# zlib-ng/minizip-ng

Hardware: AMD Instinct MI355X
Metric: decompressed GiB/s (whole node) + CRC32 match rate, 100k x 64KiB DEFLATE entries (higher is better)
Workload: dtype u8

## Files before the change

minizip-ng_amd/csrc/crc32_core.h:

```cpp
#ifndef MZHIP_CRC32_CORE_H
#define MZHIP_CRC32_CORE_H

#include <stddef.h>
#include "wave.h"

#define MZ_CRC_POLY 0xEDB88320u
#define MZ_CRC_TILE 1024u
#define MZ_CRC_SUPER 4096u

typedef struct mzhip_crc_tables {
    uint32_t byte_tab[256];
    uint32_t kx[32];
    uint32_t x16[64];
    uint32_t x1[16];
    uint32_t kx4[32];
    uint32_t x64[64];
    uint32_t mul4[4][256];
    uint32_t slice[4][256];
} mzhip_crc_tables;

static inline uint32_t mzhip_gf2_mul_host(uint32_t a, uint32_t b) {
    uint32_t p = 0;
    for (int i = 0; i < 32; i++) {
        if (a & 0x80000000u) p ^= b;
        a <<= 1;
        b = (b & 1) ? ((b >> 1) ^ MZ_CRC_POLY) : (b >> 1);
    }
    return p;
}
static inline uint32_t mzhip_xpow8_host(uint64_t nbytes) {
    uint32_t r = 0x80000000u, sq = 0x00800000u;
    while (nbytes) {
        if (nbytes & 1) r = mzhip_gf2_mul_host(r, sq);
        sq = mzhip_gf2_mul_host(sq, sq);
        nbytes >>= 1;
    }
    return r;
}
static inline void mzhip_crc_tables_init(mzhip_crc_tables *t) {
    for (uint32_t n = 0; n < 256; n++) {
        uint32_t c = n;
        for (int k = 0; k < 8; k++) c = (c & 1) ? (MZ_CRC_POLY ^ (c >> 1)) : (c >> 1);
        t->byte_tab[n] = c;
    }
    uint32_t k = mzhip_xpow8_host(MZ_CRC_TILE - 16);
    for (int j = 0; j < 32; j++) {
        t->kx[j] = k;
        k = (k & 1) ? ((k >> 1) ^ MZ_CRC_POLY) : (k >> 1);
    }
    for (int j = 0; j < 64; j++) t->x16[j] = mzhip_xpow8_host(16u * (uint32_t)j);
    for (int j = 0; j < 16; j++) t->x1[j] = mzhip_xpow8_host((uint32_t)j);
    k = mzhip_xpow8_host(MZ_CRC_SUPER - 64);
    for (int j = 0; j < 32; j++) {
        t->kx4[j] = k;
        k = (k & 1) ? ((k >> 1) ^ MZ_CRC_POLY) : (k >> 1);
    }
    for (int j = 0; j < 64; j++) t->x64[j] = mzhip_xpow8_host(64u * (uint32_t)j);
    for (int b = 0; b < 4; b++)
        for (uint32_t n = 0; n < 256; n++) t->mul4[b][n] = mzhip_gf2_mul_host(n << (8 * b), t->kx4[0]);
    for (uint32_t n = 0; n < 256; n++) t->slice[0][n] = t->byte_tab[n];
    for (int k2 = 1; k2 < 4; k2++)
        for (uint32_t n = 0; n < 256; n++) t->slice[k2][n] = (t->slice[k2 - 1][n] >> 8) ^ t->byte_tab[t->slice[k2 - 1][n] & 255];
}
static inline uint32_t mzhip_crc32_combine_host(uint32_t crc_a, uint32_t crc_b, uint64_t len_b) {
    return mzhip_gf2_mul_host(mzhip_xpow8_host(len_b), crc_a) ^ crc_b;
}

MZ_DEV uint32_t mz_gf2_mul(uint32_t a, uint32_t b) {
    uint32_t p = 0;
#pragma unroll 4
    for (int i = 0; i < 32; i++) {
        p ^= b & (0u - (a >> 31));
        a <<= 1;
        b = (b >> 1) ^ (MZ_CRC_POLY & (0u - (b & 1)));
    }
    return p;
}

MZ_DEV uint32_t mz_gf2_mul_kx(uint32_t a, const uint32_t *kx) {
    uint32_t p = 0;
#pragma unroll
    for (int j = 0; j < 32; j++)
        p ^= kx[j] & (0u - ((a >> (31 - j)) & 1u));
    return p;
}

MZ_DEV uint32_t mz_load_u32(const uint8_t *p) {
    uint32_t v;
    __builtin_memcpy(&v, p, 4);
    return v;
}

MZ_DEV uint32_t mz_crc_dword(uint32_t r, uint32_t d, const uint32_t *tab) {
    r ^= d;
    r = tab[r & 255] ^ (r >> 8);
    r = tab[r & 255] ^ (r >> 8);
    r = tab[r & 255] ^ (r >> 8);
    r = tab[r & 255] ^ (r >> 8);
    return r;
}

#define MZ_CRC_FOLD_TILES(acc, done, buf, upto, tab, kx)                                   \
    while ((uint64_t)(done) + MZ_CRC_TILE <= (uint64_t)(upto)) {                           \
        MZ_LANES {                                                                         \
            const uint8_t *_p = (buf) + (done) + 16u * (uint32_t)lane;                     \
            uint32_t _r = P(acc);                                                          \
            if ((done) != 0) _r = mz_gf2_mul_kx(_r, (kx));      \
            _r = mz_crc_dword(_r, mz_load_u32(_p), (tab));                                 \
            _r = mz_crc_dword(_r, mz_load_u32(_p + 4), (tab));                             \
            _r = mz_crc_dword(_r, mz_load_u32(_p + 8), (tab));                             \
            _r = mz_crc_dword(_r, mz_load_u32(_p + 12), (tab));                            \
            P(acc) = _r;                                                                   \
        }                                                                                  \
        (done) += MZ_CRC_TILE;                                                             \
    }

MZ_DEV uint32_t mz_crc_dword4(uint32_t r, uint32_t d, const uint32_t *tab4) {
    const uint32_t x = r ^ d;
    return tab4[768u + (x & 255u)] ^ tab4[512u + ((x >> 8) & 255u)] ^ tab4[256u + ((x >> 16) & 255u)] ^ tab4[x >> 24];
}

#define MZ_CRC_FOLD_SUPER(acc, done, buf, n, tab4, mul4)                                    \
    while ((uint64_t)(done) + MZ_CRC_SUPER <= (uint64_t)(n)) {                             \
        MZ_LANES {                                                                         \
            const uint8_t *_p = (buf) + (done) + 64u * (uint32_t)lane;                     \
            uint32_t _r = P(acc);                                                          \
            if ((done) != 0)  \
                _r = (mul4)[_r & 255u] ^ (mul4)[256u + ((_r >> 8) & 255u)] ^ (mul4)[512u + ((_r >> 16) & 255u)] ^ (mul4)[768u + (_r >> 24)]; \
            for (int _k = 0; _k < 4; _k++) {                                               \
                uint32_t _q[4];                                                            \
                __builtin_memcpy(_q, _p + 16 * _k, 16);              \
                _r = mz_crc_dword4(_r, _q[0], (tab4));                                     \
                _r = mz_crc_dword4(_r, _q[1], (tab4));                                     \
                _r = mz_crc_dword4(_r, _q[2], (tab4));                                     \
                _r = mz_crc_dword4(_r, _q[3], (tab4));                                     \
            }                                                                              \
            P(acc) = _r;                                                                   \
        }                                                                                  \
        (done) += MZ_CRC_SUPER;                                                            \
    }
#define MZ_CRC_ADVANCE_SUPER(r, kxp) mz_crc_advance_gm((r), (const uint32_t *)((const uint8_t *)(kxp) + (offsetof(mzhip_crc_tables, mul4) - offsetof(mzhip_crc_tables, kx4))))
MZ_DEV uint32_t mz_crc_advance_gm(uint32_t r, const uint32_t *mul4) {
    return mul4[r & 255u] ^ mul4[256u + ((r >> 8) & 255u)] ^ mul4[512u + ((r >> 16) & 255u)] ^ mul4[768u + (r >> 24)];
}
#define MZ_CRC_FOLD_SUPER_BT(acc, done, buf, upto, tab, kx4)                               \
    while ((uint64_t)(done) + MZ_CRC_SUPER <= (uint64_t)(upto)) {                          \
        MZ_LANES {                                                                         \
            const uint8_t *_p = (buf) + (done) + 64u * (uint32_t)lane;                     \
            uint32_t _r = P(acc);                                                          \
            if ((done) != 0) _r = MZ_CRC_ADVANCE_SUPER(_r, (kx4));                         \
            for (int _k = 0; _k < 4; _k++) {                                               \
                uint32_t _q[4];                                                            \
                __builtin_memcpy(_q, _p + 16 * _k, 16);              \
                _r = mz_crc_dword(_r, _q[0], (tab));                                       \
                _r = mz_crc_dword(_r, _q[1], (tab));                                       \
                _r = mz_crc_dword(_r, _q[2], (tab));                                       \
                _r = mz_crc_dword(_r, _q[3], (tab));                                       \
            }                                                                              \
            P(acc) = _r;                                                                   \
        }                                                                                  \
        (done) += MZ_CRC_SUPER;                                                            \
    }
#define MZ_CRC_FINISH_SUPER_BT(result, acc, tmp, done, buf, n, tab, tabs)                  \
    do {                                                                                   \
        uint32_t _sreg = 0xFFFFFFFFu;                                                      \
        if ((done) != 0) {                                                                 \
            MZ_CRC_SUPER_REDUCE(_sreg, acc, tmp, tabs);                                    \
        }                                                                                  \
        const uint8_t *_rest = (buf) + (done);                                             \
        const uint32_t _nrest = (uint32_t)((n) - (done));                                  \
        uint32_t _rdone = 0;                                                               \
        MZ_LANES { P(acc) = (lane == 0) ? _sreg : 0u; }                                    \
        MZ_CRC_FOLD_TILES(acc, _rdone, _rest, _nrest, tab, (tabs)->kx);                    \
        MZ_CRC_FINISH_FROM(result, acc, tmp, _rdone, _rest, _nrest, tab, tabs, _sreg);     \
    } while (0)
#define MZ_CRC_SUPER_REDUCE(reg, acc, tmp, tabs)                                           \
    do {                                                                                   \
        MZ_LANES { P(tmp) = mz_gf2_mul(P(acc), (tabs)->x64[63 - lane]); }                  \
        MZ_WAVE_XOR(reg, tmp);                                                             \
    } while (0)

#define MZ_CRC_FINISH_FROM(result, acc, tmp, done, buf, n, tab, tabs, reg0)                \
    do {                                                                                   \
        uint32_t _reg = (reg0);                                                            \
        if ((done) != 0) {                                                                 \
            MZ_LANES { P(tmp) = mz_gf2_mul(P(acc), (tabs)->x16[63 - lane]); }              \
            MZ_WAVE_XOR(_reg, tmp);                                                        \
        }                                                                                  \
        uint32_t _r = (uint32_t)((n) - (done));                    \
        if (_r != 0) {                                                                     \
            MZ_LANES {                                                                     \
                uint32_t _o = 16u * (uint32_t)lane;                                        \
                uint32_t _v = _r > _o ? (_r - _o > 16u ? 16u : _r - _o) : 0u;              \
                uint32_t _c = (lane == 0) ? _reg : 0u;                                     \
                const uint8_t *_p = (buf) + (done) + _o;                                   \
                for (uint32_t _i = 0; _i < _v; _i++)                                       \
                    _c = (tab)[(_c ^ _p[_i]) & 255] ^ (_c >> 8);                           \
                uint32_t _rem = _r - _o - _v;           \
                if (_v == 0) { _c = 0; _rem = 0; }                                         \
                _c = mz_gf2_mul(_c, (tabs)->x16[_rem >> 4]);                               \
                _c = mz_gf2_mul(_c, (tabs)->x1[_rem & 15]);                                \
                P(tmp) = _c;                                                               \
            }                                                                              \
            MZ_WAVE_XOR(_reg, tmp);                                                        \
        }                                                                                  \
        (result) = ~_reg;                                                                  \
    } while (0)

#define MZ_CRC_FINISH(result, acc, tmp, done, buf, n, tab, tabs) \
    MZ_CRC_FINISH_FROM(result, acc, tmp, done, buf, n, tab, tabs, 0xFFFFFFFFu)

#endif
```

minizip-ng_amd/csrc/inflate_commit.inc:

```
{
    MZ_WAVE_SYNC();
    uint8_t *const gdst = out + out_pos;
    MZ_STAT(10, Tb); MZ_STAT(12, Tm); MZ_STAT(15, 1);
    {
        uint64_t badm;
        MZ_BALLOT(badm, P(bad) != 0u);
        if (badm) fail = 1;
    }
    uint32_t nnear = 0;
    for (uint32_t b = 0; b < Tm && !fail; b += 64u) {
        PV(uint32_t, e0);
        PV(uint32_t, rem);
        MZ_LANES {
            mz_piece32 pc;
            const uint32_t j = b + (uint32_t)lane;
            uint32_t en = 0, rm = 0, nf = 0, si = 0;
            if (j < Tm) {
                en = lst[-(int32_t)(j + 1u)];
                si = en & 0xFFFu;
                const uint32_t ln = mz_bfe(en, 12, 5) + 1u, dist = (en >> 17) + 1u;
                const uint32_t dstw = si - sb;
                if (dist > dstw) {
                    nf = dist - dstw;
                    if (nf > ln) nf = ln;
// ... 47 lines not shown
            }
            P(d0) = a;
            P(rem) = rm;
            P(dist) = ds;
            P(kst) = rm ? a : 0xFFFFFFFFu;
            P(ken) = rm ? a + rm : 0xFFFFFFFFu;
            P(ca) = 0u;
            P(cb) = 0u;
        }
#pragma unroll
        for (uint32_t step = 32u; step != 0u; step >>= 1) {
            PV(uint32_t, va);
            PV(uint32_t, vb);
            MZ_GATHER(va, ken, P(ca) + step - 1u);
            MZ_GATHER(vb, kst, P(cb) + step - 1u);
            MZ_LANES {
                const uint32_t s0 = P(d0) - P(dist), s1 = s0 + ((P(rem) < P(dist)) ? P(rem) : P(dist));
                if (P(va) <= s0) P(ca) += step;
                if (P(vb) < s1) P(cb) += step;
            }
        }
        MZ_LANES {
            P(dep) = (P(cb) > P(ca)) ? ((~0ull >> (64u - (P(cb) - P(ca)))) << P(ca)) : 0ull;
        }
        uint64_t U;
        MZ_BALLOT(U, P(rem) != 0u);
        MZ_STAT_ZERO(11);
        while (U) {
            MZ_STAT(14, 1); MZ_STAT(11, 1); MZ_STAT_MAX(24, 11);
            uint64_t R;
            MZ_BALLOT(R, P(rem) != 0u && (P(dep) & U) == 0ull);
            if (!R) {
                MZ_STAT(22, 1);
                fail = 1;
                break;
            }
            MZ_LANES {
                if (P(rem) != 0u && (P(dep) & U) == 0ull) {
                    uint8_t *d = stg + P(d0);
                    uint32_t n = P(rem), D = P(dist);
                    if (D < 8u) {
                        const uint32_t D8 = D * ((7u + D) / D);
                        uint32_t pro = D8 - D;
                        if (pro > n) pro = n;
                        for (uint32_t k = 0; k < pro; k++) d[k] = d[(int32_t)k - (int32_t)D];
                        d += pro;
                        n -= pro;
                        D = D8;
                    }
                    mz_copy32_seq(d, d - D, n);
                    P(rem) = 0u;
                }
            }
            MZ_WAVE_SYNC();
            U &= ~R;
        }
    }
#endif
    MZ_PROF_MARK(7);
    if (!fail) {
#if !(MZ_ABLATE & 8)
        {
            const uint32_t e = sb + Tb;
            const uint32_t a0 = sb ? 16u : 0u, a1 = e & ~15u;
            uint8_t *const gal = gdst - sb;
            const uint32_t hn = ((a0 < e) ? a0 : e) - sb;
            const uint32_t t0 = (a1 > a0) ? a1 : a0;
            const uint32_t tn = (e > t0) ? e - t0 : 0u;
            MZ_LANES {
                if ((uint32_t)lane < hn) gal[sb + (uint32_t)lane] = stg[sb + (uint32_t)lane];
                if ((uint32_t)lane < tn) gal[t0 + (uint32_t)lane] = stg[t0 + (uint32_t)lane];
                for (uint32_t c = a0 + 16u * (uint32_t)lane; c + 16u <= a1; c += 1024u) {
                    const uint64_t v0 = mz_ld8(stg + c), v1 = mz_ld8(stg + c + 8u);
                    mz_st8(gal + c, v0);
                    mz_st8(gal + c + 8u, v1);
                }
            }
        }
#endif
        MZ_WAVE_SYNC();
        out_pos += Tb;
        MZ_PROF_MARK(8);
#if !(MZ_ABLATE & 4)
        MZ_CRC_FOLD_SUPER_BT(crc_acc, crc_done, out + crc_base, out_pos - crc_base, crc_tab, tabs->kx4);
#endif
        MZ_PROF_MARK(9);
    }
}
```

minizip-ng_amd/csrc/inflate_core.h:

```cpp
#ifndef MZHIP_INFLATE_CORE_H
#define MZHIP_INFLATE_CORE_H
#if defined(MZ_STATS)
extern unsigned long long mz_stats[32], mz_stat_max;
#define MZ_STAT(i, v) (mz_stats[i] += (v))
#define MZ_STAT_ZERO(i) (mz_stats[i] = 0)
#define MZ_STAT_MAX(i, j) (mz_stats[i] = mz_stats[j] > mz_stats[i] ? mz_stats[j] : mz_stats[i])
#define MZ_STAT_LANE(v) (mz_stat_max = (v) > mz_stat_max ? (v) : mz_stat_max)
#define MZ_STAT_LANEMAX(i) (mz_stats[i] += mz_stat_max, mz_stat_max = 0)
#else
#define MZ_STAT(i, v) ((void)0)
#define MZ_STAT_ZERO(i) ((void)0)
#define MZ_STAT_MAX(i, j) ((void)0)
#define MZ_STAT_LANE(v) ((void)0)
#define MZ_STAT_LANEMAX(i) ((void)0)
#endif

#include "crc32_core.h"
#include "wave.h"
#if defined(MZ_PROF) && !defined(MZHIP_HOST_EMUL)
extern __device__ unsigned long long mz_prof_buf[32];
#define MZ_PROF_DECL                     \
    uint32_t prof_acc = 0;  \
    uint64_t prof_t0 = __builtin_readcyclecounter();
#define MZ_PROF_MARK(i)                                                           \
// ... 200 lines not shown
    for (int k = root + 1; k < 15; k++) len += (v15 >= lim[k]) ? 1u : 0u;
    const uint32_t idx = (uint32_t)((int32_t)delta[len] + (int32_t)(v15 >> (15u - len)));
    const uint32_t ok = (v15 < lim[15] && idx < nent) ? 1u : 0u;
    const uint32_t e = ent[ok ? idx : 0u];
    return ok ? e + len : 0u;
}

#define MZ_HDR_WIN_BITS(dst, pos_)                                                            \
    do {                                                                                      \
        const uint32_t _ab = (pos_) + 8u * in_mis, _j = (_ab >> 5) - hw0;                     \
        if (_j + 2u < 64u) {                                                                  \
            const uint32_t _d0 = MZ_READLANE(hwin, _j), _d1 = MZ_READLANE(hwin, _j + 1u), _d2 = MZ_READLANE(hwin, _j + 2u); \
            const uint32_t _s = _ab & 31u;                                                    \
            uint64_t _v = (((uint64_t)_d1 << 32) | _d0) >> _s;                                \
            if (_s) _v |= (uint64_t)_d2 << (64u - _s);                                        \
            (dst) = _v;                                                                       \
        } else {                                                                              \
            (dst) = mz_bits_at(in, in_len, (pos_));                                           \
        }                                                                                     \
    } while (0)

#define MZ_HDR_BITS(dst, n)                                                   \
    do {                                                                      \
        if (bitpos + (uint32_t)(n) > total_bits) {                            \
            status = MZHIP_BUF_ERROR;                                         \
            goto finish;                                                      \
        }                                                                     \
        uint64_t _w;                                                          \
        MZ_HDR_WIN_BITS(_w, bitpos);                                          \
        (dst) = MZ_UNIFORM((uint32_t)_w & ((1u << (n)) - 1));                 \
        bitpos += (n);                                                        \
    } while (0)

MZ_DEV uint32_t mz_load_stream_dword(const uint8_t *in_al, uint32_t in_mis, uint32_t in_len, uint32_t j) {
    const uint64_t lo = (uint64_t)j * 4u, end = (uint64_t)in_mis + in_len;
    if (lo >= end) return 0u;
    uint32_t d = *(const uint32_t *)(in_al + lo);
    if (lo < in_mis) d &= 0xFFFFFFFFu << (8u * (in_mis - (uint32_t)lo));
    if (lo + 4u > end) d &= 0xFFFFFFFFu >> (8u * (uint32_t)(lo + 4u - end));
    return d;
}

#if defined(MZHIP_HOST_EMUL)
static const uint8_t mz_k_order[19] = {16, 17, 18, 0, 8, 7, 9, 6, 10, 5, 11, 4, 12, 3, 13, 2, 14, 1, 15};
#else
__device__ static const uint8_t mz_k_order[19] = {16, 17, 18, 0, 8, 7, 9, 6, 10, 5, 11, 4, 12, 3, 13, 2, 14, 1, 15};
#endif


MZ_DEV void mz_bitrange(uint32_t sh, uint32_t n, uint32_t *m0, uint32_t *m1) {
    const uint32_t full = 0xFFFFFFFFu >> (32u - n);
    *m0 = full << sh;
    *m1 = (full >> 1) >> (31u - sh);
}
typedef struct {
    uint64_t v[4];
    uint32_t t4, t2, t1;
} mz_piece32;
MZ_DEV void mz_copy32_load(mz_piece32 *r, const uint8_t *src, uint32_t n) {
    const uint32_t n8 = n & ~7u;
    r->v[0] = r->v[1] = r->v[2] = r->v[3] = 0;
    r->t4 = r->t2 = r->t1 = 0;
#pragma unroll
    for (uint32_t k = 0; k < 4u; k++)
        if (8u * k + 8u <= n) r->v[k] = mz_ld8(src + 8u * k);
    if (n & 4u) r->t4 = mz_ld4(src + n8);
    if (n & 2u) r->t2 = mz_ld2(src + n8 + (n & 4u));
    if (n & 1u) r->t1 = src[n - 1u];
}
MZ_DEV void mz_copy32_store(const mz_piece32 *r, uint8_t *dst, uint32_t n) {
    const uint32_t n8 = n & ~7u;
#pragma unroll
    for (uint32_t k = 0; k < 4u; k++)
        if (8u * k + 8u <= n) mz_st8(dst + 8u * k, r->v[k]);
    if (n & 4u) mz_st4(dst + n8, r->t4);
    if (n & 2u) mz_st2(dst + n8 + (n & 4u), (uint16_t)r->t2);
    if (n & 1u) dst[n - 1u] = (uint8_t)r->t1;
}
MZ_DEV void mz_copy32(uint8_t *dst, const uint8_t *src, uint32_t n) {
    mz_piece32 r;
    mz_copy32_load(&r, src, n);
    mz_copy32_store(&r, dst, n);
}
MZ_DEV void mz_copy32_seq(uint8_t *dst, const uint8_t *src, uint32_t n) {
    const uint32_t n8 = n & ~7u;
#pragma unroll
    for (uint32_t k = 0; k < 4u; k++)
        if (8u * k + 8u <= n) mz_st8(dst + 8u * k, mz_ld8(src + 8u * k));
    if (n & 4u) mz_st4(dst + n8, mz_ld4(src + n8));
    if (n & 2u) mz_st2(dst + n8 + (n & 4u), mz_ld2(src + n8 + (n & 4u)));
    if (n & 1u) dst[n - 1u] = src[n - 1u];
}

#define MZ_K_LIT 0x40u
#define MZ_K_EOB 0x80u
MZ_DEV uint32_t mz_chase_step(const mz_inflate_lds *L, uint32_t d0, uint32_t d1, uint32_t d2, uint32_t rel, uint32_t room,
                              uint32_t *rec) {
    uint32_t w0 = mz_funnel(d1, d0, rel), w1 = mz_funnel(d2, d1, rel);
    uint32_t e = L->lit_fast[w0 & ((1u << MZ_LROOT) - 1u)];
    if (e & MZ_E_SUB) e = L->lit_sub[((e >> 8) & 0x1FFu) + mz_bfe(w0, MZ_LROOT, e & 7u)];
    uint32_t r = 0, pb = 0;
    if ((((e & (MZ_E_LEN | 0x80u)) == 0x80u) & ((e & 63u) < room)) != 0) {
        pb = e & 63u;
        r = 0x80000000u | mz_bfe(e, 16, 8);
        w0 = mz_funnel(w1, w0, pb);
        w1 >>= pb;
        e = L->lit_fast[w0 & ((1u << MZ_LROOT) - 1u)];
        if (e & MZ_E_SUB) e = L->lit_sub[((e >> 8) & 0x1FFu) + mz_bfe(w0, MZ_LROOT, e & 7u)];
    }
    if (!(e & MZ_E_LEN)) {
        const uint32_t nb = e & 63u;
        *rec = r | ((e >> 8) & 0xFF00u);
        return nb ? ((nb + pb) | ((e & 0x80u) ? MZ_K_LIT : MZ_K_EOB)) : 0u;
    }
    const uint32_t nb = e & 63u, ex = mz_bfe(e, 16, 4);
    const uint32_t lenl = mz_bfe(e, 7, 9) + mz_bfe(mz_funnel(w1, w0, nb), 0, ex);
    const uint32_t nb2 = nb + ex;
    const uint32_t dl = mz_funnel(w1, w0, nb2);
    uint32_t dd = L->dist_fast[dl & ((1u << MZ_DROOT) - 1u)];
    MZ_STAT(19, 1);
    if (dd == 0u) {
        MZ_STAT(20, 1);
        dd = mz_long_code(dl, MZ_DROOT, L->dist_lim, L->dist_delta, L->dist_ent, 32u);
    }
    if ((int32_t)dd <= 0) {
        *rec = 0u;
        return 0u;
    }
    const uint32_t dn = dd & 15u, dex = mz_bfe(dd, 4, 4);
    const uint32_t dist = mz_bfe(dd, 8, 15) + mz_bfe(dl, dn, dex);
    *rec = r | ((lenl - 3u) << 8) | ((dist - 1u) << 16);
    return nb2 + dn + dex + pb;
}
typedef struct { uint32_t v[4]; } mz_dw4;
MZ_DEV mz_dw4 mz_load_stream_dw4(const uint8_t *in_al, uint32_t in_mis, uint32_t in_len, uint32_t d) {
    mz_dw4 r;
    const uint64_t lo = (uint64_t)d * 4u, end = (uint64_t)in_mis + in_len;
    if (lo >= in_mis && lo + 16u <= end) {
        __builtin_memcpy(&r, in_al + lo, 16);
    } else {
#pragma unroll
        for (uint32_t k = 0; k < 4u; k++) r.v[k] = mz_load_stream_dword(in_al, in_mis, in_len, d + k);
    }
    return r;
}


#include "inflate_walk.inc"
#include "inflate_emit.inc"

typedef struct mz_inflate_par {
    uint32_t mode;
    uint32_t *ptr;
} mz_inflate_par;
#define MZHIP_PAR_BAIL (-301)

MZ_DEV uint32_t mz_block_header_plausible(const uint8_t *in, uint32_t in_len, uint32_t p) {
    if ((uint64_t)(p >> 3) + 24u > in_len) return 0u;
    uint64_t w = mz_bits_at(in, in_len, p);
    const uint32_t h = (uint32_t)w;
    if (((h >> 1) & 3u) == 0u) {
        const uint32_t b = (p + 3u + 7u) >> 3;
        const uint32_t len = (uint32_t)in[b] | ((uint32_t)in[b + 1] << 8), nlen = (uint32_t)in[b + 2] | ((uint32_t)in[b + 3] << 8);
        return (len ^ nlen) == 0xFFFFu ? 1u : 0u;
    }
    if (((h >> 1) & 3u) != 2u) return 0u;
    if (((h >> 3) & 31u) > 29u || ((h >> 8) & 31u) > 29u) return 0u;
    const uint32_t ncode = ((h >> 13) & 15u) + 4u;
    uint32_t kraft = 0;
    w >>= 17;
    for (uint32_t i = 0; i < ncode; i++) {
        if (i == 15u) w = mz_bits_at(in, in_len, p + 17u + 45u);
        const uint32_t l = (uint32_t)w & 7u;
        w >>= 3;
// ... 40 lines not shown
        if (_adv <= in_rem) {                                          \
            in += _adv;                                                \
            in_al += _adv;                                             \
            in_adv += _adv;                                            \
            in_rem -= _adv;                                            \
            in_len = in_rem < MZ_VIEW_MAX ? in_rem : MZ_VIEW_MAX;      \
            total_bits = in_len * 8u;                                  \
            bitpos -= _adv * 8u;                                       \
            MZ_EDGE_GROUPS();                                          \
            also;                                                      \
        }                                                              \
    }
    uint32_t out_pos = rs ? MZ_UNIFORM(rs->out_pos) : 0u;
    uint32_t chase_smax = MZ_CHASE_SMAX;
    int32_t status = MZHIP_OK;
    uint32_t last = 0;
    PV(uint32_t, crc_acc);
    PV(uint32_t, crc_tmp);
    const uint32_t crc_base = out_pos;
    uint32_t crc_done = 0;
    MZ_LANES { P(crc_acc) = (lane == 0) ? 0xFFFFFFFFu : 0u; }
    MZ_PROF_DECL

    while (!last) {
        if (par && par_blocks) goto finish;
        MZ_REBASE((void)0)
        hdr_bit = bitpos;
        in_header = 1;
        if (stop_at_header && par_blocks) {
            status = MZHIP_OUT_FULL;
            goto finish;
        }
        const uint32_t hw0 = (bitpos + 8u * in_mis) >> 5;
        PV(uint32_t, hwin);
        MZ_LANES { P(hwin) = mz_load_stream_dword(in_al, in_mis, in_len, hw0 + (uint32_t)lane); }
        uint32_t hdr;
        MZ_HDR_BITS(hdr, 3);
        last = hdr & 1u;
        uint32_t btype = hdr >> 1;

        if (btype == 0) {
            uint32_t byte = (uint32_t)((bitpos + 7) >> 3);
            if ((uint64_t)byte + 4 > in_len) {
                status = MZHIP_BUF_ERROR;
                goto finish;
            }
            uint32_t len = MZ_UNIFORM((uint32_t)in[byte] | ((uint32_t)in[byte + 1] << 8));
            uint32_t nlen = MZ_UNIFORM((uint32_t)in[byte + 2] | ((uint32_t)in[byte + 3] << 8));
            byte += 4;
            bitpos = byte * 8u;
            if (len != (~nlen & 0xFFFFu)) {
                status = MZHIP_DATA_ERROR;
                goto finish;
            }
            uint32_t avail = in_len - byte;
            uint32_t n = len < avail ? len : avail;
            if (resumable && n < len) {
                status = MZHIP_BUF_ERROR;
                goto finish;
            }
            if (n > out_cap - out_pos) {
                status = MZHIP_OUT_FULL;
                goto finish;
            }
            if (par && n < len) {
                status = MZHIP_PAR_BAIL;
                goto finish;
            }
            if (!par || par->mode == 2u) {
                MZ_LANES {
                    for (uint32_t i = (uint32_t)lane; i < n; i += 64) {
                        out[out_pos + i] = in[byte + i];
                        if (par) par->ptr[out_pos + i] = out_pos + i;
                    }
                }
                MZ_WAVE_SYNC();
            }
            out_pos += n;
            bitpos += n * 8u;
            if (n < len) {
                status = MZHIP_BUF_ERROR;
                goto finish;
            }
            if (!par) MZ_CRC_FOLD_SUPER_BT(crc_acc, crc_done, out + crc_base, out_pos - crc_base, crc_tab, tabs->kx4);
            in_header = 0;
            hdr_bit = bitpos;
            par_blocks++;
            continue;
        }
        if (btype == 3) {
            status = MZHIP_DATA_ERROR;
            goto finish;
        }

        uint32_t sub_used;
        {
            const mz_code_result cr = mz_block_code(MZ_LDS_HANDLE(L), MZ_GLB_HANDLE(in), in_len, in_mis, total_bits, bitpos, hw0, btype, hwin MZ_PROF_ARGS);
            sub_used = MZ_UNIFORM(cr.sub_used);
            bitpos = MZ_UNIFORM(cr.bitpos);
            if (MZ_UNIFORM(cr.status) != (uint32_t)MZHIP_OK) {
                status = (int32_t)MZ_UNIFORM(cr.status);
                goto finish;
            }
        }
        in_header = 0;
        if (resume_at != 0xFFFFFFFFu) {
            if (resume_at > bitpos) bitpos = resume_at;
            resume_at = 0xFFFFFFFFu;
        }
        {
            uint32_t *ring = MZ_L_RING(L);
            const uint32_t pbase = 8u * in_mis;
            uint32_t ring_hi = 0;
            uint32_t ring_valid = 0;
            PV(uint32_t, wpre);

            PV(uint32_t, tq);
            uint32_t qn = 0;
            MZ_LANES { P(tq) = 0u; }

            uint32_t span_skip = 0;
            uint32_t span_on = (use_span && rec) ? 1u : 0u;
            for (;;) {
                MZ_REBASE(ring_valid = 0)
                {
                    const uint32_t remain = total_bits - bitpos;
                    if (span_on && qn == 0u && !span_skip && remain >= 64u + 2u * 128u) {
                        ring_valid = 0;
                        MZ_PROF_MARK(3);
#include "inflate_chase.inc"
                    }
                    if (par) {
                        status = MZHIP_PAR_BAIL;
                        goto finish;
                    }
                    span_skip = 0;
                }
                if (!ring_valid) {
                    const uint32_t blk = (bitpos + pbase) >> 11;
                    MZ_LANES {
                        const uint32_t da = mz_load_stream_dword(in_al, in_mis, in_len, blk * 64u + (uint32_t)lane);
                        const uint32_t db = mz_load_stream_dword(in_al, in_mis, in_len, (blk + 1u) * 64u + (uint32_t)lane);
                        ring[((blk & 1u) << 6) + (uint32_t)lane] = da;
                        ring[(((blk + 1u) & 1u) << 6) + (uint32_t)lane] = db;
                        if (lane < 2) ring[128 + lane] = (blk & 1u) ? db : da;
                        P(wpre) = mz_load_stream_dword(in_al, in_mis, in_len, (blk + 2u) * 64u + (uint32_t)lane);
                    }
                    ring_hi = blk + 2u;
                    ring_valid = 1;
                    MZ_WAVE_SYNC();
                }
                if (qn == 0u) qbit = bitpos;
                const uint32_t pbit = bitpos + pbase;
                if ((pbit >> 11) + 1u >= ring_hi) {
                    MZ_LANES {
                        ring[((ring_hi & 1u) << 6) + (uint32_t)lane] = P(wpre);
                        if (lane < 2 && !(ring_hi & 1u)) ring[128 + lane] = P(wpre);
                        P(wpre) = mz_load_stream_dword(in_al, in_mis, in_len, (ring_hi + 1u) * 64u + (uint32_t)lane);
                    }
                    ring_hi++;
                    MZ_WAVE_SYNC();
                }

                PV(uint32_t, w0);
                PV(uint32_t, w1);
                PV(uint32_t, le);
                MZ_LANES {
// ... 218 lines not shown
```

minizip-ng_amd/csrc/inflate_emit.inc:

```
#define MZ_EMIT_LOAD_GROUP(G0_) \
        MZ_LANES { \
            const uint32_t G = (G0_) + (uint32_t)lane; \
            uint32_t lo = 0, hi_ = 0, st0 = 0; \
            uint32_t kw0 = 0, kw1 = 0; \
_Pragma("unroll") \
            for (uint32_t k = 0; k < MZ_EMIT_GROUP; k++) P(w)[k] = 0u; \
            if (G < NG) { \
                uint32_t j = 0;  \
_Pragma("unroll") \
                for (uint32_t sp = 32u; sp; sp >>= 1) \
                    if (tab_g[j + sp - 1u] <= G) j += sp; \
                const uint32_t k = G - (j ? tab_g[j - 1u] : 0u); \
                const uint32_t n = tab_n[j], e = tab_e[j], m = tab_m[j]; \
                const uint32_t ts = e & 0x7FFFu; \
                const uint32_t cr = (n > ts) ? ((n + MZ_EMIT_GROUP - 1u) / MZ_EMIT_GROUP) - ts / MZ_EMIT_GROUP : 0u; \
                const uint8_t *base, *kbase; \
                if (k < cr) {  \
                    st0 = (ts / MZ_EMIT_GROUP + k) * MZ_EMIT_GROUP; \
                    lo = (ts > st0) ? ts : st0; \
                    hi_ = (n < st0 + MZ_EMIT_GROUP) ? n : st0 + MZ_EMIT_GROUP; \
                    base = Rp; \
                    kbase = Lp + j * MZ_REC_CAP1; \
                } else { \
                    st0 = (k - cr) * MZ_EMIT_GROUP; \
                    lo = st0; \
                    hi_ = (m < st0 + MZ_EMIT_GROUP) ? m : st0 + MZ_EMIT_GROUP; \
                    base = Cp; \
                    kbase = Lc + j * MZ_REC_CAP2; \
                } \
_Pragma("unroll") \
                for (uint32_t pp = 0; pp < MZ_EMIT_GROUP / 4u; pp++) { \
                    mz_dw4 v; \
                    __builtin_memcpy(&v, base + MZ_REC_ADDR(st0 / 4u + pp, j), 16); \
                    P(w)[4u * pp] = v.v[0]; \
                    P(w)[4u * pp + 1u] = v.v[1]; \
                    P(w)[4u * pp + 2u] = v.v[2]; \
                    P(w)[4u * pp + 3u] = v.v[3]; \
                } \
                { \
                    const uint64_t kk = mz_ld8(kbase + st0); \
                    kw0 = (uint32_t)kk; \
                    kw1 = (uint32_t)(kk >> 32); \
                } \
            } \
             \
_Pragma("unroll") \
            for (uint32_t r = 0; r < MZ_EMIT_GROUP; r++) { \
                const uint32_t st = st0 + r; \
                const uint32_t kb = mz_bfe((r & 4u) ? kw1 : kw0, 8u * (r & 3u), 8); \
                const uint32_t in = (st >= lo && st < hi_ && kb != 0u) ? 1u : 0u; \
                const uint32_t ln = (kb < MZ_K_LIT) ? mz_bfe(P(w)[r], 8, 8) + 3u : (kb < MZ_K_EOB) ? 1u : 0u; \
                P(w)[r] = in ? P(w)[r] : 0u; \
                P(kq)[r] = in ? ((kb & 63u) | (ln << 8)) : 0u; \
            } \
        }

typedef struct mz_emit_result {
    uint32_t out_pos, crc_done;
    uint32_t cbits;
    uint32_t fail;
    uint32_t all;
    PV(uint32_t, crc_acc);
} mz_emit_result;
MZ_DEV_NOINLINE mz_emit_result mz_chase_emit(mz_lds_handle L_, uint32_t sub_used_, mz_glb_handle rec_, mz_glb_handle out_, uint32_t out_pos_,
                                             uint32_t out_cap_, uint32_t NG_, uint32_t crc_base_, uint32_t crc_done_, PVIN(uint32_t, crc_acc_in),
                                             mz_lds_handle crc_tab_, mz_glb_handle tabs_ MZ_PROF_PARAMS) {
    MZ_LANE_DECL
    const uint32_t sub_used = MZ_UNIFORM(sub_used_), out_cap = MZ_UNIFORM(out_cap_), NG = MZ_UNIFORM(NG_), crc_base = MZ_UNIFORM(crc_base_);
    uint32_t out_pos = MZ_UNIFORM(out_pos_), crc_done = MZ_UNIFORM(crc_done_);
    mz_inflate_lds *const L = MZ_LDS_FROM(mz_inflate_lds, L_);
    uint8_t *const rec = MZ_GLB_FROM(uint8_t, rec_);
    uint8_t *const out = MZ_GLB_FROM(uint8_t, out_);
    const uint32_t *const crc_tab = MZ_LDS_FROM(const uint32_t, crc_tab_);
    const mzhip_crc_tables *const tabs = MZ_GLB_FROM(const mzhip_crc_tables, tabs_);
    PV(uint32_t, crc_acc);
    MZ_LANES { P(crc_acc) = P(crc_acc_in); }
    uint32_t *const pool0 = L->lit_sub + ((sub_used + 3u) & ~3u);
    uint8_t *const stg = (uint8_t *)pool0;
    uint32_t *const ring = MZ_L_WIN(L);
    uint32_t *const tab_n = ring + 64u * MZ_CRING_RS - 256u, *const tab_e = tab_n + 64, *const tab_m = tab_n + 128, *const tab_g = tab_n + 192;
    uint32_t *const lst = tab_n;
    const uint32_t pool_bytes = (uint32_t)((uint8_t *)lst - stg);
    uint8_t *const Rp = rec;
    uint8_t *const Cp = rec + MZ_REC_AREA(MZ_REC_CAP1);
    uint8_t *const Lp = Cp + MZ_REC_AREA(MZ_REC_CAP2);
    uint8_t *const Lc = Lp + 64u * MZ_REC_CAP1;
    uint32_t G0 = 0;
    uint32_t cbits = 0;
    uint32_t fail = 0;
    PV(uint32_t, bad);
    while (G0 < NG) {
        MZ_STAT(9, 1);
        const uint32_t sb = (uint32_t)((uintptr_t)(out + out_pos) & 15u);
        PV2(uint32_t, w, MZ_EMIT_GROUP);
        PV2(uint32_t, kq, MZ_EMIT_GROUP);
        MZ_EMIT_LOAD_GROUP(G0)
#define MZ_CHASE_REC(r_, in_, rc_, ln_)                                                      \
        const uint32_t rc_ = P(w)[(r_)];                                                     \
        const uint32_t in_ = P(kq)[(r_)] ? 1u : 0u;                                          \
        const uint32_t ln_ = P(kq)[(r_)] >> 8;
        PV(uint32_t, lby);
        PV(uint32_t, lpc);
        PV(uint32_t, lbt);
        MZ_LANES {
            uint32_t by = 0, pc = 0, bt = 0;
#pragma unroll
            for (uint32_t r = 0; r < MZ_EMIT_GROUP; r++) {
                MZ_CHASE_REC(r, in, rc, ln)
                (void)in;
                by += ln + (rc >> 31);
                pc += (ln > 1u) ? (ln + 31u) >> 5 : 0u;
                bt += P(kq)[r] & 63u;
            }
            P(lby) = by;
            P(lpc) = pc;
            P(lbt) = bt;
        }
        PV(uint32_t, sib);
        PV(uint32_t, sim);
        MZ_INCL_SCAN(sib, lby);
        MZ_INCL_SCAN(sim, lpc);
#define MZ_CHASE_FITS(B_, M_) ((B_) <= 4096u && (B_) + 4u * (M_) + 48u <= pool_bytes)
        uint64_t nofit;
        MZ_BALLOT(nofit, !MZ_CHASE_FITS(sb + P(sib), P(sim)));
        const uint32_t cut = nofit ? mz_ctz64(nofit) : 64u;
        PV(uint32_t, acc);
        uint32_t Tb, Tm, Tbits;
        MZ_LANES {
            P(acc) = ((uint32_t)lane < cut) ? MZ_EMIT_GROUP : 0u;
            if ((uint32_t)lane >= cut) P(lbt) = 0u;
        }
        Tb = MZ_READLANE(sib, (cut ? cut : 1u) - 1u);
        Tm = MZ_READLANE(sim, (cut ? cut : 1u) - 1u);
#undef MZ_CHASE_FITS
        MZ_WAVE_SUM(Tbits, lbt);
        if (cut == 0u || Tbits == 0u || Tb > out_cap - out_pos) {
            fail = 1;
            break;
        }
        uint64_t longm;
        MZ_LANES {
            uint32_t bd = 0;
            uint32_t pos = sb + P(sib) - P(lby), mi = P(sim) - P(lpc);
#pragma unroll
            for (uint32_t r = 0; r < MZ_EMIT_GROUP; r++) {
                MZ_CHASE_REC(r, in, rc, ln)
                if (in && r < P(acc)) {
                    if (rc >> 31) stg[pos++] = (uint8_t)rc;
                    if (ln == 1u) {
                        stg[pos] = (uint8_t)(rc >> 8);
                    } else if (ln > 1u) {
                        const uint32_t dist = mz_bfe(rc, 16, 15) + 1u;
                        bd |= (dist > out_pos + (pos - sb)) ? 1u : 0u;
                        lst[-(int32_t)(mi + 1u)] = pos | ((((ln < 32u) ? ln : 32u) - 1u) << 12) | ((dist - 1u) << 17);
                        mi += (ln + 31u) >> 5;
                    }
                    pos += ln;
                }
            }
            P(bad) = bd;
        }
        {
            PV(uint32_t, lng);
            MZ_LANES {
                uint32_t m = 0;
#pragma unroll
                for (uint32_t r = 0; r < MZ_EMIT_GROUP; r++) m |= ((P(kq)[r] >> 8) > 32u) ? 1u : 0u;
                P(lng) = (P(acc) != 0u) ? m : 0u;
            }
            MZ_BALLOT(longm, P(lng) != 0u);
        }
        if (longm) {
            MZ_LANES {
                uint32_t pos = sb + P(sib) - P(lby), mi = P(sim) - P(lpc);
#pragma unroll
                for (uint32_t r = 0; r < MZ_EMIT_GROUP; r++) {
                    MZ_CHASE_REC(r, in, rc, ln)
                    if (in && r < P(acc)) {
                        pos += rc >> 31;
                        if (ln > 1u) {
                            const uint32_t dist = mz_bfe(rc, 16, 15) + 1u;
                            MZ_NOUNROLL
                            for (uint32_t o = 32u; o < ln; o += 32u)
                                lst[-(int32_t)(mi + (o >> 5) + 1u)] = (pos + o) | ((((ln - o < 32u) ? ln - o : 32u) - 1u) << 12) | ((dist - 1u) << 17);
                            mi += (ln + 31u) >> 5;
                        }
                        pos += ln;
                    }
                }
            }
        }
#undef MZ_CHASE_REC
        MZ_PROF_MARK(13);
#include "inflate_commit.inc"
        if (fail) break;
        cbits += Tbits;
        G0 += cut;
    }
    mz_emit_result er;
    er.out_pos = out_pos;
    er.crc_done = crc_done;
    er.cbits = cbits;
    er.fail = fail;
    er.all = (G0 >= NG) ? 1u : 0u;
    MZ_LANES { P(er.crc_acc) = P(crc_acc); }
    return er;
}

// ... 73 lines not shown
```

minizip-ng_amd/csrc/inflate_flush.inc:

```
{
        PV(uint32_t, olen);
        PV(uint32_t, oend);
        MZ_LANES {
            if ((uint32_t)lane >= qn) P(tq) = 0u;
            P(olen) = mz_bfe(P(tq), 7, 9);
        }
        MZ_STAT(4, qn);
        MZ_STAT(6, 1);
        qn = 0;
        MZ_INCL_SCAN(oend, olen);
        uint32_t total = MZ_READLANE(oend, 63);
        uint32_t part_bits = 0;
        if (total > out_cap - out_pos) {
            uint64_t over_m, far_m;
            MZ_BALLOT(over_m, P(oend) > out_cap - out_pos);
            MZ_BALLOT(far_m, P(olen) > 1u && (P(tq) >> 16) > out_pos + P(oend) - P(olen));
            const uint32_t fo = mz_ctz64(over_m);
            const uint32_t far_first = (far_m & ((fo >= 63u) ? ~0ull : ((2ull << fo) - 1ull))) ? 1u : 0u;
            if (far_first || !resumable || par || fo == 0u) {
                status = far_first ? MZHIP_DATA_ERROR : MZHIP_OUT_FULL;
                unwritten = 1;
                goto finish;
            }
            PV(uint32_t, tb);
// ... 12 lines not shown
        }
        uint64_t matm;
        MZ_BALLOT(matm, P(olen) > 1u);
        {
            MZ_LANES {
                if (P(olen) == 1u) out[out_pos + P(oend) - 1u] = (uint8_t)(P(tq) >> 16);
            }
            MZ_WAVE_SYNC();

            if (matm) {
                const uint32_t nmatch = mz_popc64(matm);
                uint32_t done_m = 0;
                MZ_LANES {
                    if (P(olen) > 1u) MZ_L_MSLOT(L)[mz_popc64(matm & ((1ull << lane) - 1ull))] = (uint16_t)(4 * lane);
                }
                MZ_WAVE_SYNC();
                MZ_STAT(0, 1); MZ_STAT(1, nmatch);
                while (done_m < nmatch) {
                    MZ_STAT(2, 1);
                    PV(uint32_t, msrc);
                    PV(uint32_t, mtk);
                    PV(uint32_t, mend);
                    MZ_LANES {
                        const uint32_t g = done_m + ((uint32_t)lane >> MZ_MLANES_LOG2);
                        P(msrc) = (g < nmatch) ? (uint32_t)MZ_L_MSLOT(L)[g] : 256u;
                    }
                    MZ_GATHER4(mtk, tq, P(msrc));
                    MZ_GATHER4(mend, oend, P(msrc));
                    MZ_LANES {
                        if (P(msrc) >= 256u) { P(mtk) = 0; P(mend) = 0; }
                    }
                    const uint32_t gs = MZ_READLANE(mend, 0) - mz_bfe(MZ_READLANE(mtk, 0), 7, 9);
                    uint64_t dep;
                    MZ_BALLOT(dep, P(mend) > (P(mtk) >> 16) + gs ||
                                       (P(mtk) >> 16) > out_pos + P(mend) - mz_bfe(P(mtk), 7, 9));
                    const uint32_t nind = dep ? (mz_ctz64(dep) >> MZ_MLANES_LOG2) : (64u >> MZ_MLANES_LOG2);
                    if (nind) {
                        MZ_LANES {
                            if (P(msrc) < 256u && ((uint32_t)lane >> MZ_MLANES_LOG2) < nind) {
                                const uint32_t ln = mz_bfe(P(mtk), 7, 9), dist = P(mtk) >> 16;
                                const uint32_t dst = out_pos + P(mend) - ln;
                                for (uint32_t i = (uint32_t)lane & ((1u << MZ_MLANES_LOG2) - 1u); i < ln; i += 1u << MZ_MLANES_LOG2)
                                    out[dst + i] = out[dst - dist + i];
                            }
                        }
                        MZ_WAVE_SYNC();
                        done_m += nind;
                    }
                    if (dep && done_m < nmatch) {
                        MZ_STAT(3, 1);
                        const uint32_t tl = MZ_UNIFORM(MZ_L_MSLOT(L)[done_m]) >> 2;
                        const uint32_t t = MZ_READLANE(tq, tl);
                        const uint32_t ln = (t >> 7) & 511u, dist = t >> 16;
                        const uint32_t dst = out_pos + MZ_READLANE(oend, tl) - ln;
                        if (dist > dst) {
                            status = MZHIP_DATA_ERROR;
                            out_pos = dst;
                            {
                                PV(uint32_t, tb);
                                PV(uint32_t, te);
                                MZ_LANES { P(tb) = P(tq) & 63u; }
                                MZ_INCL_SCAN(te, tb);
                                bitpos = qbit + MZ_READLANE(te, tl);
                            }
                            goto finish;
                        }
                        const uint8_t *src = out + (dst - dist);
                        if (dist >= ln) {
                            MZ_LANES {
                                for (uint32_t i = (uint32_t)lane; i < ln; i += 64u) out[dst + i] = src[i];
                            }
                        } else {
                            MZ_LANES {
                                for (uint32_t i = (uint32_t)lane; i < ln; i += 64u) out[dst + i] = src[i % dist];
                            }
                        }
                        MZ_WAVE_SYNC();
                        done_m++;
                    }
                }
            }
        }
        out_pos += total;
        MZ_CRC_FOLD_SUPER_BT(crc_acc, crc_done, out + crc_base, out_pos - crc_base, crc_tab, tabs->kx4);
        if (part_bits) {
            bitpos = qbit + part_bits;
            status = MZHIP_OUT_FULL;
            goto finish;
        }
}
```

Before: 382.9.

## Interleave multiple independent CRC chains per super-tile and add optional emit prefetch

The CRC super-tile fold now processes two 4 KiB super-tiles at once as independent per-lane chains. The table lookups of the chains interleave, which hides the latency of the serial byte-table dependency. The chains are merged with a new precomputed x^(8*4096) multiply table. The change also adds two experimental paths that are off by default: software prefetch of the next emit group, and a different tail copy for short sequential copies. The multi-chain fold raises register pressure and only kicks in when at least 8 KiB is pending, so a larger remainder goes through the slower finish path.

```diff
diff --git a/minizip-ng_amd/csrc/crc32_core.h b/minizip-ng_amd/csrc/crc32_core.h
--- a/minizip-ng_amd/csrc/crc32_core.h
+++ b/minizip-ng_amd/csrc/crc32_core.h
@@ -17,6 +17,7 @@
     uint32_t x64[64];
     uint32_t mul4[4][256];
     uint32_t slice[4][256];
+    uint32_t mul4k[4][256];
 } mzhip_crc_tables;
 
 static inline uint32_t mzhip_gf2_mul_host(uint32_t a, uint32_t b) {
@@ -58,6 +59,9 @@
     for (int j = 0; j < 64; j++) t->x64[j] = mzhip_xpow8_host(64u * (uint32_t)j);
     for (int b = 0; b < 4; b++)
         for (uint32_t n = 0; n < 256; n++) t->mul4[b][n] = mzhip_gf2_mul_host(n << (8 * b), t->kx4[0]);
+    k = mzhip_xpow8_host(MZ_CRC_SUPER);
+    for (int b = 0; b < 4; b++)
+        for (uint32_t n = 0; n < 256; n++) t->mul4k[b][n] = mzhip_gf2_mul_host(n << (8 * b), k);
     for (uint32_t n = 0; n < 256; n++) t->slice[0][n] = t->byte_tab[n];
     for (int k2 = 1; k2 < 4; k2++)
         for (uint32_t n = 0; n < 256; n++) t->slice[k2][n] = (t->slice[k2 - 1][n] >> 8) ^ t->byte_tab[t->slice[k2 - 1][n] & 255];
@@ -161,6 +165,56 @@
         }                                                                                  \
         (done) += MZ_CRC_SUPER;                                                            \
     }
+#ifndef MZ_CRC_CHAINS
+#define MZ_CRC_CHAINS 2
+#endif
+#if MZ_CRC_CHAINS != 1 && MZ_CRC_CHAINS != 2 && MZ_CRC_CHAINS != 4
+#error "MZ_CRC_CHAINS must be 1, 2 or 4"
+#endif
+#if MZ_CRC_CHAINS == 4
+#define MZ_CRC_GROUP_UNR MZ_NOUNROLL
+#else
+#define MZ_CRC_GROUP_UNR
+#endif
+#define MZ_CRC_GROUP_LB 16u
+#define MZ_CRC_ADVANCE_SUPER4K(r, kxp) mz_crc_advance_gm((r), (const uint32_t *)((const uint8_t *)(kxp) + (offsetof(mzhip_crc_tables, mul4k) - offsetof(mzhip_crc_tables, kx4))))
+#if MZ_CRC_CHAINS == 1
+#define MZ_CRC_FOLD_SUPER_BT_GROUP(acc, done, buf, upto, tab, kx4) MZ_CRC_FOLD_SUPER_BT(acc, done, buf, upto, tab, kx4)
+#else
+#define MZ_CRC_FOLD_SUPER_BT_GROUP(acc, done, buf, upto, tab, kx4)                         \
+    while ((uint64_t)(done) + MZ_CRC_CHAINS * MZ_CRC_SUPER <= (uint64_t)(upto)) {          \
+        MZ_LANES {                                                                         \
+            const uint8_t *_p = (buf) + (done) + 64u * (uint32_t)lane;                     \
+            uint32_t _c[MZ_CRC_CHAINS];                                                    \
+            _c[0] = P(acc);                                                                \
+            if ((done) != 0) _c[0] = MZ_CRC_ADVANCE_SUPER(_c[0], (kx4));                   \
+_Pragma("unroll")                                                                          \
+            for (int _i = 1; _i < MZ_CRC_CHAINS; _i++) _c[_i] = 0u;                        \
+            MZ_CRC_GROUP_UNR                                                               \
+            for (uint32_t _k = 0; _k < 64u; _k += MZ_CRC_GROUP_LB) {                       \
+                uint32_t _q[MZ_CRC_CHAINS][MZ_CRC_GROUP_LB / 4u];                          \
+_Pragma("unroll")                                                                          \
+                for (int _i = 0; _i < MZ_CRC_CHAINS; _i++)                                 \
+                    __builtin_memcpy(_q[_i], _p + MZ_CRC_SUPER * (uint32_t)_i + _k, MZ_CRC_GROUP_LB);  \
+_Pragma("unroll")                                                                          \
+                for (uint32_t _d = 0; _d < MZ_CRC_GROUP_LB / 4u; _d++) {                   \
+_Pragma("unroll")                                                                          \
+                    for (int _i = 0; _i < MZ_CRC_CHAINS; _i++) _c[_i] ^= _q[_i][_d];       \
+_Pragma("unroll")                                                                          \
+                    for (int _b = 0; _b < 4; _b++)                                         \
+_Pragma("unroll")                                                                          \
+                        for (int _i = 0; _i < MZ_CRC_CHAINS; _i++)  \
+                            _c[_i] = (tab)[_c[_i] & 255u] ^ (_c[_i] >> 8);                 \
+                }                                                                          \
+            }                                                                              \
+            uint32_t _r = _c[0];                                                           \
+_Pragma("unroll")                                                                          \
+            for (int _i = 1; _i < MZ_CRC_CHAINS; _i++) _r = MZ_CRC_ADVANCE_SUPER4K(_r, (kx4)) ^ _c[_i]; \
+            P(acc) = _r;                                                                   \
+        }                                                                                  \
+        (done) += MZ_CRC_CHAINS * MZ_CRC_SUPER;                                            \
+    }
+#endif
 #define MZ_CRC_FINISH_SUPER_BT(result, acc, tmp, done, buf, n, tab, tabs)                  \
     do {                                                                                   \
         uint32_t _sreg = 0xFFFFFFFFu;                                                      \
diff --git a/minizip-ng_amd/csrc/inflate_commit.inc b/minizip-ng_amd/csrc/inflate_commit.inc
--- a/minizip-ng_amd/csrc/inflate_commit.inc
+++ b/minizip-ng_amd/csrc/inflate_commit.inc
@@ -153,7 +153,7 @@
         out_pos += Tb;
         MZ_PROF_MARK(8);
 #if !(MZ_ABLATE & 4)
-        MZ_CRC_FOLD_SUPER_BT(crc_acc, crc_done, out + crc_base, out_pos - crc_base, crc_tab, tabs->kx4);
+        MZ_CRC_FOLD_SUPER_BT_GROUP(crc_acc, crc_done, out + crc_base, out_pos - crc_base, crc_tab, tabs->kx4);
 #endif
         MZ_PROF_MARK(9);
     }
diff --git a/minizip-ng_amd/csrc/inflate_core.h b/minizip-ng_amd/csrc/inflate_core.h
--- a/minizip-ng_amd/csrc/inflate_core.h
+++ b/minizip-ng_amd/csrc/inflate_core.h
@@ -306,7 +306,29 @@
     mz_copy32_load(&r, src, n);
     mz_copy32_store(&r, dst, n);
 }
+#ifndef MZ_NEAR_TAIL
+#define MZ_NEAR_TAIL 0
+#endif
 MZ_DEV void mz_copy32_seq(uint8_t *dst, const uint8_t *src, uint32_t n) {
+#if MZ_NEAR_TAIL
+    uint64_t v0 = 0;
+    uint32_t t4 = 0, t2 = 0, t1 = 0;
+    if (n >= 8u) v0 = mz_ld8(src);
+    if (n < 8u && (n & 4u)) t4 = mz_ld4(src);
+    if (n < 8u && (n & 2u)) t2 = mz_ld2(src + (n & 4u));
+    if (n < 8u && (n & 1u)) t1 = src[n - 1u];
+    if (n >= 8u) {
+        mz_st8(dst, v0);
+#pragma unroll
+        for (uint32_t k = 1; k < 4u; k++)
+            if (8u * k + 8u <= n) mz_st8(dst + 8u * k, mz_ld8(src + 8u * k));
+        if (n & 7u) mz_st8(dst + (n - 8u), mz_ld8(src + (n - 8u)));
+    } else {
+        if (n & 4u) mz_st4(dst, t4);
+        if (n & 2u) mz_st2(dst + (n & 4u), t2);
+        if (n & 1u) dst[n - 1u] = (uint8_t)t1;
+    }
+#else
     const uint32_t n8 = n & ~7u;
 #pragma unroll
     for (uint32_t k = 0; k < 4u; k++)
@@ -314,6 +336,7 @@
     if (n & 4u) mz_st4(dst + n8, mz_ld4(src + n8));
     if (n & 2u) mz_st2(dst + n8 + (n & 4u), mz_ld2(src + n8 + (n & 4u)));
     if (n & 1u) dst[n - 1u] = src[n - 1u];
+#endif
 }
 
 #define MZ_K_LIT 0x40u
@@ -520,7 +543,7 @@
                 status = MZHIP_BUF_ERROR;
                 goto finish;
             }
-            if (!par) MZ_CRC_FOLD_SUPER_BT(crc_acc, crc_done, out + crc_base, out_pos - crc_base, crc_tab, tabs->kx4);
+            if (!par) MZ_CRC_FOLD_SUPER_BT_GROUP(crc_acc, crc_done, out + crc_base, out_pos - crc_base, crc_tab, tabs->kx4);
             in_header = 0;
             hdr_bit = bitpos;
             par_blocks++;
diff --git a/minizip-ng_amd/csrc/inflate_emit.inc b/minizip-ng_amd/csrc/inflate_emit.inc
--- a/minizip-ng_amd/csrc/inflate_emit.inc
+++ b/minizip-ng_amd/csrc/inflate_emit.inc
@@ -1,10 +1,21 @@
 #define MZ_EMIT_LOAD_GROUP(G0_) \
+        { \
+            PV2(uint32_t, fw_, MZ_EMIT_GROUP); \
+            PV(uint32_t, fk0_); \
+            PV(uint32_t, fk1_); \
+            PV(uint32_t, flo_); \
+            PV(uint32_t, fhi_); \
+            PV(uint32_t, fst_); \
+            MZ_EMIT_FETCH_GROUP(G0_, fw_, fk0_, fk1_, flo_, fhi_, fst_) \
+            MZ_EMIT_MASK_GROUP(fw_, fk0_, fk1_, flo_, fhi_, fst_) \
+        }
+#define MZ_EMIT_FETCH_GROUP(G0_, fw, fk0, fk1, flo, fhi, fst) \
         MZ_LANES { \
             const uint32_t G = (G0_) + (uint32_t)lane; \
             uint32_t lo = 0, hi_ = 0, st0 = 0; \
             uint32_t kw0 = 0, kw1 = 0; \
 _Pragma("unroll") \
-            for (uint32_t k = 0; k < MZ_EMIT_GROUP; k++) P(w)[k] = 0u; \
+            for (uint32_t k = 0; k < MZ_EMIT_GROUP; k++) P(fw)[k] = 0u; \
             if (G < NG) { \
                 uint32_t j = 0;  \
 _Pragma("unroll") \
@@ -32,10 +43,10 @@
                 for (uint32_t pp = 0; pp < MZ_EMIT_GROUP / 4u; pp++) { \
                     mz_dw4 v; \
                     __builtin_memcpy(&v, base + MZ_REC_ADDR(st0 / 4u + pp, j), 16); \
-                    P(w)[4u * pp] = v.v[0]; \
-                    P(w)[4u * pp + 1u] = v.v[1]; \
-                    P(w)[4u * pp + 2u] = v.v[2]; \
-                    P(w)[4u * pp + 3u] = v.v[3]; \
+                    P(fw)[4u * pp] = v.v[0]; \
+                    P(fw)[4u * pp + 1u] = v.v[1]; \
+                    P(fw)[4u * pp + 2u] = v.v[2]; \
+                    P(fw)[4u * pp + 3u] = v.v[3]; \
                 } \
                 { \
                     const uint64_t kk = mz_ld8(kbase + st0); \
@@ -43,17 +54,28 @@
                     kw1 = (uint32_t)(kk >> 32); \
                 } \
             } \
+            P(fk0) = kw0; \
+            P(fk1) = kw1; \
+            P(flo) = lo; \
+            P(fhi) = hi_; \
+            P(fst) = st0; \
+        }
+#define MZ_EMIT_MASK_GROUP(fw, fk0, fk1, flo, fhi, fst) \
+        MZ_LANES { \
              \
 _Pragma("unroll") \
             for (uint32_t r = 0; r < MZ_EMIT_GROUP; r++) { \
-                const uint32_t st = st0 + r; \
-                const uint32_t kb = mz_bfe((r & 4u) ? kw1 : kw0, 8u * (r & 3u), 8); \
-                const uint32_t in = (st >= lo && st < hi_ && kb != 0u) ? 1u : 0u; \
-                const uint32_t ln = (kb < MZ_K_LIT) ? mz_bfe(P(w)[r], 8, 8) + 3u : (kb < MZ_K_EOB) ? 1u : 0u; \
-                P(w)[r] = in ? P(w)[r] : 0u; \
+                const uint32_t st = P(fst) + r; \
+                const uint32_t kb = mz_bfe((r & 4u) ? P(fk1) : P(fk0), 8u * (r & 3u), 8); \
+                const uint32_t in = (st >= P(flo) && st < P(fhi) && kb != 0u) ? 1u : 0u; \
+                const uint32_t ln = (kb < MZ_K_LIT) ? mz_bfe(P(fw)[r], 8, 8) + 3u : (kb < MZ_K_EOB) ? 1u : 0u; \
+                P(w)[r] = in ? P(fw)[r] : 0u; \
                 P(kq)[r] = in ? ((kb & 63u) | (ln << 8)) : 0u; \
             } \
         }
+#ifndef MZ_EMIT_PREFETCH
+#define MZ_EMIT_PREFETCH 0
+#endif
 
 typedef struct mz_emit_result {
     uint32_t out_pos, crc_done;
@@ -89,12 +111,25 @@
     uint32_t cbits = 0;
     uint32_t fail = 0;
     PV(uint32_t, bad);
+#if MZ_EMIT_PREFETCH
+    PV2(uint32_t, nw, MZ_EMIT_GROUP);
+    PV(uint32_t, nk0);
+    PV(uint32_t, nk1);
+    PV(uint32_t, nlo);
+    PV(uint32_t, nhi);
+    PV(uint32_t, nst);
+    MZ_EMIT_FETCH_GROUP(G0, nw, nk0, nk1, nlo, nhi, nst)
+#endif
     while (G0 < NG) {
         MZ_STAT(9, 1);
         const uint32_t sb = (uint32_t)((uintptr_t)(out + out_pos) & 15u);
         PV2(uint32_t, w, MZ_EMIT_GROUP);
         PV2(uint32_t, kq, MZ_EMIT_GROUP);
+#if MZ_EMIT_PREFETCH
+        MZ_EMIT_MASK_GROUP(nw, nk0, nk1, nlo, nhi, nst)
+#else
         MZ_EMIT_LOAD_GROUP(G0)
+#endif
 #define MZ_CHASE_REC(r_, in_, rc_, ln_)                                                      \
         const uint32_t rc_ = P(w)[(r_)];                                                     \
         const uint32_t in_ = P(kq)[(r_)] ? 1u : 0u;                                          \
@@ -124,6 +159,9 @@
         uint64_t nofit;
         MZ_BALLOT(nofit, !MZ_CHASE_FITS(sb + P(sib), P(sim)));
         const uint32_t cut = nofit ? mz_ctz64(nofit) : 64u;
+#if MZ_EMIT_PREFETCH
+        MZ_EMIT_FETCH_GROUP(G0 + cut, nw, nk0, nk1, nlo, nhi, nst)
+#endif
         PV(uint32_t, acc);
         uint32_t Tb, Tm, Tbits;
         MZ_LANES {
diff --git a/minizip-ng_amd/csrc/inflate_flush.inc b/minizip-ng_amd/csrc/inflate_flush.inc
--- a/minizip-ng_amd/csrc/inflate_flush.inc
+++ b/minizip-ng_amd/csrc/inflate_flush.inc
@@ -118,7 +118,7 @@
             }
         }
         out_pos += total;
-        MZ_CRC_FOLD_SUPER_BT(crc_acc, crc_done, out + crc_base, out_pos - crc_base, crc_tab, tabs->kx4);
+        MZ_CRC_FOLD_SUPER_BT_GROUP(crc_acc, crc_done, out + crc_base, out_pos - crc_base, crc_tab, tabs->kx4);
         if (part_bits) {
             bitpos = qbit + part_bits;
             status = MZHIP_OUT_FULL;
```

After: 402.8, median of 6. +5.2%, better.
